# guo-research-group/Blurry-Edges

Hardware: AMD Instinct MI355X
Metric: patch-pairs/s (local CNN + render + depth) on 21x21 synth (higher is better)
Workload: dtype f32; 1 GPU; configs[1]: batch of 4096 synthetic 21x21 two-aperture patch pairs per GPU (8192 CNN patches): LocalStage inference + pass-A colour solve + depth solve; pairs_per_gpu=4096, streams=2, weights=portable-generator random init (no checkpoint offline)

## Files before the change

### blurry-edges_amd/be_hip/native.py

```python
from __future__ import annotations

import ctypes as C
import os

import torch

_HERE = os.path.dirname(os.path.abspath(__file__))
_ALT_DIR = os.environ.get("BE_LIB_DIR")
LIB_PATH = os.path.join(_ALT_DIR or os.path.join(os.path.dirname(_HERE), "lib"), "libblurry_edges_hip.so")

BE_R = 21
NPIX = 441
NTENSORS = 86


class PackJob(C.Structure):
    _fields_ = [("weight", C.c_void_p), ("bias", C.c_void_p), ("bn_gamma", C.c_void_p), ("bn_beta", C.c_void_p),
                ("bn_mean", C.c_void_p), ("bn_var", C.c_void_p), ("packed_w", C.c_void_p), ("packed_bias", C.c_void_p),
                ("bn_eps", C.c_float), ("cout", C.c_int), ("cin", C.c_int), ("ksize", C.c_int), ("layout_chw_hw", C.c_int),
                ("dgrad", C.c_int)]


class AdamEntry(C.Structure):
    _fields_ = [("p", C.c_void_p), ("m", C.c_void_p), ("v", C.c_void_p), ("goff", C.c_int64), ("n", C.c_int)]
# ... 57 lines not shown
    "be_conv_nhwc_splitk_f32": (C.c_int, [C.POINTER(ConvDesc), _P, _P, _P, _P, _P, C.c_int, _P, C.c_size_t, _P]),
    "be_conv_nhwc_batched_f32": (C.c_int, [C.POINTER(ConvDesc), _P, _P, _P, _P, C.c_int, C.c_int, C.c_int64, C.c_int64, C.c_int64, _P]),
    "be_wino_tile_rows": (C.c_int, []),
    "be_wino_packed_floats": (C.c_size_t, [C.c_int, C.c_int]),
    "be_wino_pack_f32": (C.c_int, [_P] * 6 + [C.c_float, C.c_int, C.c_int, _P, _P, _P]),
    "be_wino_workspace_floats": (C.c_size_t, [C.c_int64, C.c_int, C.c_int]),
    "be_wino_conv3x3_6x6_f32": (C.c_int, [_P] * 5 + [C.c_int64, C.c_int, C.c_int, C.c_int, _P, C.c_size_t, _P]),
    "be_gemm_rows_bf6_packed_floats": (C.c_size_t, [C.c_int, C.c_int]),
    "be_gemm_rows_bf6_pack_f32": (C.c_int, [_P, C.c_int, C.c_int, _P, _P]),
    "be_gemm_rows_bf6_f32": (C.c_int, [_P, C.c_int64, C.c_int, _P, C.c_int, _P, _P, C.c_int, _P, C.c_int, _P]),
    "be_conv3x3_pm_bf6_packed_floats": (C.c_size_t, [C.c_int, C.c_int, C.c_int]),
    "be_conv3x3_pm_bf6_pack_f32": (C.c_int, [_P, C.c_int, C.c_int, C.c_int, _P, _P]),
    "be_conv3x3_pm_bf6_f32": (C.c_int, [C.POINTER(ConvDesc), _P, _P, C.c_int, _P, _P, _P, C.c_int, _P]),
    "be_wino_pair_workspace_floats": (C.c_size_t, [C.c_int64, C.c_int, C.c_int, C.c_int]),
    "be_wino_conv3x3_pair_6x6_f32": (C.c_int, [_P, _P, _P, C.c_int, _P, _P, _P, C.c_int, _P, C.c_int64, C.c_int, C.c_int, C.c_int, _P,
                                               C.c_size_t, _P]),
    "be_conv_fused2_packed_floats": (C.c_size_t, [C.c_int] * 4),
    "be_conv_pack_fused2_f32": (C.c_int, [_P] * 12 + [C.c_float] + [C.c_int] * 4 + [_P, _P, _P]),
    "be_conv_nhwc_fused2_f32": (C.c_int, [C.POINTER(ConvDesc), _P, _P, C.c_int, _P, _P, _P, C.c_int, _P]),
    "be_maxpool_nhwc_f32": (C.c_int, [_P, _P] + [C.c_int] * 7 + [_P]),
    "be_eval_depth_f32": (C.c_int, [_P, _P, _P] + [C.c_int] * 4 + [C.c_float] * 3 + [_P, _P]),
    "be_maxpool_nhwc_ld_f32": (C.c_int, [_P, C.c_int, _P] + [C.c_int] * 7 + [_P]),
    "be_nchw_to_nhwc_pad_f32": (C.c_int, [_P, _P, C.c_int64, C.c_int, C.c_int64, C.c_int, _P]),
    "be_upconv2x2_scatter_f32": (C.c_int, [_P, _P, C.c_int64] + [C.c_int] * 9 + [_P]),
    "be_datagen_raster_words": (C.c_size_t, [C.c_int] * 4),
    "be_datagen_raster_u32": (C.c_int, [_P, _P] + [C.c_int] * 4 + [_P, _P]),
    "be_datagen_scene_f64": (C.c_int, [_P, _P, _P, _P] + [C.c_int] * 4 + [C.c_double] + [_P] * 5),
    "be_datagen_blur_scratch_bytes": (C.c_size_t, [C.c_int] * 3),
    "be_datagen_blur_composite_f64": (C.c_int, [_P] * 5 + [C.c_int] * 5 + [_P, _P, C.c_size_t, _P]),
    "be_datagen_finish_f64": (C.c_int, [_P] * 4 + [C.c_int] * 3 + [_P, C.c_size_t, _P]),
    "be_datagen_noise_f64": (C.c_int, [_P, _P, C.c_double, C.c_uint32, C.c_int64, C.c_int64, _P, _P, _P]),
    "be_datagen_candidates_f64": (C.c_int, [_P, _P] + [C.c_int] * 5 + [_P]),
    "be_datagen_crop_f64": (C.c_int, [_P, _P, _P, _P, _P, C.c_int64] + [C.c_int] * 4 + [_P, _P]),
    "be_datagen_test_psf_doubles": (C.c_size_t, [C.c_int] * 3),
    "be_datagen_test_render_f64": (C.c_int, [_P] * 8 + [C.c_size_t] + [C.c_int] * 6 + [_P, _P, _P]),
    "be_attention_train_workspace_floats": (C.c_size_t, [C.c_int, C.c_int, C.c_int]),
    "be_attention_train_fwd_f32": (C.c_int, [_P, _P, _P, _P, C.c_int, C.c_int, C.c_int, C.c_int, C.c_float, C.c_uint32, _P]),
    "be_attention_bwd_scratch_floats": (C.c_size_t, [C.c_int, C.c_int, C.c_int]),
    "be_attention_bwd_f32": (C.c_int, [_P, _P, _P, _P, _P, _P, _P, C.c_int, C.c_int, C.c_int, C.c_int, C.c_int, C.c_float, C.c_uint32, _P]),
    "be_attention_dropout_mask_f32": (C.c_int, [_P, C.c_int, C.c_int, C.c_int, C.c_float, C.c_uint32, _P]),
    "be_attention_train_keep_offset_floats": (C.c_size_t, [C.c_int, C.c_int, C.c_int]),
    "be_attention_keep_bits_u16": (C.c_int, [_P, C.c_int, C.c_int, C.c_int, C.c_float, C.c_uint32, _P]),
    "be_dropout_f32": (C.c_int, [_P, _P, _P, C.c_int64, C.c_float, C.c_uint32, C.c_uint32, _P]),
    "be_add_layernorm_train_f32": (C.c_int, [_P, _P, _P, _P, _P, _P, C.c_int64, C.c_int, C.c_float, C.c_float, C.c_uint32,
                                             C.c_uint32, _P]),
    "be_layernorm_bwd_partial_floats": (C.c_size_t, [C.c_int64, C.c_int]),
    "be_layernorm_bwd_f32": (C.c_int, [_P, _P, _P, _P, _P, _P, C.c_int64, C.c_int, C.c_float, C.c_float, C.c_uint32,
                                       C.c_uint32, _P]),
    "be_nchw3_to_nhwc4_f32": (C.c_int, [_P, _P, C.c_int64, C.c_int, _P]),
    "be_nchw3_to_nhwc4p_f32": (C.c_int, [_P, _P, C.c_int64, C.c_int, C.c_int, C.c_int, _P]),
    "be_view_to_nhwc4p_f32": (C.c_int, [_P, C.c_int64, C.c_int64, _P, C.c_int64, C.c_int, _P]),
    "be_conv7x7_nhwc4p_f32": (C.c_int, [C.POINTER(ConvDesc), _P, C.c_int, _P, _P, _P, C.c_int, _P]),
    "be_conv7x7_pool_nhwc4p_f32": (C.c_int, [_P, C.c_int64, _P, _P, _P, _P]),
    "be_render_full_f32": (C.c_int, [C.POINTER(RenderOpts), C.POINTER(DepthConsts), C.c_float, C.c_int, _P,
                                     C.POINTER(PatchView), _P, _P, _P, _P, _P, _P, _P, C.c_int64, _P]),
    "be_fold_records_f32": (C.c_int, [C.POINTER(RenderOpts), _P] + [C.c_int] * 6 + [_P] * 6 + [_P]),
    "be_fold_records_batch_f32": (C.c_int, [C.POINTER(RenderOpts), _P] + [C.c_int] * 7 + [_P] * 6 + [_P]),
    "be_render_full_grid_f32": (C.c_int, [C.POINTER(RenderOpts), C.POINTER(DepthConsts), C.c_float, C.c_int, _P, _P, C.c_int, C.c_int,
                                          _P, _P, C.c_int, C.c_int, _P, _P]),
    "be_fold_records_grid_f32": (C.c_int, [C.POINTER(RenderOpts), _P] + [C.c_int] * 4 + [_P, _P, C.c_int] + [_P] * 6 + [_P]),
    "be_refocus_stack_chunk": (C.c_int, []),
    "be_fold_refocus_stack_f32": (C.c_int, [C.POINTER(RenderOpts), C.POINTER(DepthConsts), _P] + [C.c_int] * 5 + [_P, _P, _P, C.c_int, _P, _P]),
    "be_fold_records_at_f32": (C.c_int, [C.POINTER(RenderOpts), _P] + [C.c_int] * 5 + [_P, _P] + [C.c_int] * 6 + [_P] * 6 + [_P]),
    "be_fold_refocus_stack_at_f32": (C.c_int, [C.POINTER(RenderOpts), C.POINTER(DepthConsts), _P] + [C.c_int] * 5 + [_P, _P] + [C.c_int] * 5
                                     + [_P, C.c_int, _P, _P]),
    "be_fold_records_points_f32": (C.c_int, [C.POINTER(RenderOpts), _P] + [C.c_int] * 5 + [_P, _P, _P, C.c_int64, C.c_int] + [_P] * 6 + [_P]),
    "be_fold_refocus_stack_points_f32": (C.c_int, [C.POINTER(RenderOpts), C.POINTER(DepthConsts), _P] + [C.c_int] * 5
                                         + [_P, _P, _P, C.c_int64, _P, C.c_int, _P, _P]),
    "be_unproject_f32": (C.c_int, [_P] + [C.c_int] * 5 + [C.POINTER(C.c_float)] * 2 + [_P, _P]),
    "be_reproject_f32": (C.c_int, [_P] + [C.c_int] * 5 + [C.POINTER(C.c_float)] * 3 + [C.c_float, C.c_int, C.c_int, _P, C.c_int] + [_P] * 4 + [_P]),
    "be_fill_nearest_f32": (C.c_int, [_P, _P, C.c_int, C.c_int, C.c_int, C.c_float, C.c_int] + [_P] * 4 + [_P]),
    "be_unfold_patches_f32": (C.c_int, [_P, _P] + [C.c_int] * 5 + [_P]),
    "be_local_features_f32": (C.c_int, [_P, _P, _P, C.c_int64, _P]),
    "be_global_denorm_f32": (C.c_int, [_P, _P, C.c_int64, _P]),
    "be_local_loss_f32": (C.c_int, [C.POINTER(RenderOpts), _P, _P, _P, _P, _P, C.c_float, C.c_float, _P, _P, _P, _P,
                                    C.c_int64, _P]),
    "be_train_scratch_bytes": (C.c_size_t, []),
    "be_bn_train_fwd_f32": (C.c_int, [_P, _P, _P, _P, C.c_float, C.c_float, _P, _P, _P, _P, _P, _P, C.c_int, C.c_int,
                                      C.c_int, _P, C.c_size_t, _P]),
    "be_bn_train_bwd_f32": (C.c_int, [_P] * 10 + [C.c_int, C.c_int, _P, C.c_size_t, _P]),
    "be_col_sum_f32": (C.c_int, [_P, _P, C.c_int, C.c_int, _P, C.c_size_t, _P]),
    "be_maxpool_nhwc_bwd_f32": (C.c_int, [_P, _P, _P] + [C.c_int] * 7 + [_P]),
    "be_conv_wgrad_f32": (C.c_int, [_P, _P, _P] + [C.c_int] * 7 + [_P, C.c_size_t, _P]),
    "be_conv_dgrad_packed_floats": (C.c_size_t, [C.c_int, C.c_int, C.c_int]),
    "be_conv_pack_dgrad_f32": (C.c_int, [_P, C.c_int, C.c_int, C.c_int, C.c_int, _P, _P, _P]),
    "be_linear_small_bwd_f32": (C.c_int, [_P] * 6 + [C.c_int] * 3 + [_P]),
    "be_adam_chunk": (C.c_int, []),
    "be_clip_adamw_f32": (C.c_int, [_P, C.c_int, _P, C.c_int64, _P, C.c_int, C.c_float, C.c_float] + [C.c_double] * 5 + [_P, _P, C.c_int, _P]),
    "be_local_loss_finish_f32": (C.c_int, [_P, C.c_int, C.c_float, C.c_float, _P, _P]),
    "be_train_unit_fwd_f32": (C.c_int, [_P] * 7 + [C.c_float, C.c_float] + [_P] * 7 + [C.c_int, _P, C.c_size_t, _P]),
    "be_train_unit_bwd_f32": (C.c_int, [_P] * 11 + [C.c_int] + [_P] * 8 + [C.c_size_t, _P]),
    "be_train_unit_pair_fwd_f32": (C.c_int, [C.POINTER(TrainUnitFwd), C.POINTER(TrainUnitFwd), C.c_float, C.c_float, _P, C.c_size_t, _P]),
    "be_train_unit_pair_bwd_f32": (C.c_int, [C.POINTER(TrainUnitBwd), C.POINTER(TrainUnitBwd), _P, C.c_size_t, _P]),
    "be_train_sk_plan_debug": (C.c_int, [C.c_int] * 7 + [C.c_double, C.POINTER(C.c_int), C.c_int]),
    "be_linear_param_grads_f32": (C.c_int, [_P, _P, _P, _P, C.c_int, C.c_int, C.c_int, _P, C.c_size_t, _P]),
    "be_linear_small_fwd_f32": (C.c_int, [_P] * 4 + [C.c_int] * 3 + [_P]),
    "be_maxpool_nhwc_fwd_idx_f32": (C.c_int, [_P, _P, _P] + [C.c_int] * 7 + [_P]),
    "be_maxpool_nhwc_bwd_idx_f32": (C.c_int, [_P, _P, _P] + [C.c_int] * 7 + [_P]),
    "be_params2dists_f32": (C.c_int, [C.POINTER(RenderOpts), _P, _P, C.c_int64, _P]),
    "be_dists2indicators_f32": (C.c_int, [_P, _P, _P, C.c_int64, _P]),
    "be_inverse3x3_f32": (C.c_int, [_P, _P, C.c_int64, _P]),
    "be_image_derivative_f32": (C.c_int, [_P, _P, C.c_int64, C.c_int, C.c_int, _P]),
    "be_fold_patches_f32": (C.c_int, [_P, _P, _P] + [C.c_int] * 7 + [C.c_int64] * 6 + [C.c_int, _P]),
    "be_params2dists_bwd_f32": (C.c_int, [C.POINTER(RenderOpts), _P, _P, _P, C.c_int64, _P]),
    "be_dists2indicators_bwd_f32": (C.c_int, [_P, _P, _P, _P, _P, C.c_int64, _P]),
    "be_inverse3x3_bwd_f32": (C.c_int, [_P, _P, _P, C.c_int64, _P]),
# ... 404 lines not shown
    check(lib().be_upconv2x2_scatter_f32(dptr(t, "t"), dptr(out, "out"), n, h, w, cout, oh, ow, (oh - 2 * h) // 2,
                                         (ow - 2 * w) // 2, ld, ch_off, stream_ptr(t.device)), "be_upconv2x2_scatter_f32")
    return out


def nchw3_to_nhwc4(x):
    n, c, h, w = x.shape
    if c != 3:
        raise RuntimeError("nchw3_to_nhwc4: expected 3 channels")
    y = torch.empty(n, h, w, 4, dtype=torch.float32, device=x.device)
    check(lib().be_nchw3_to_nhwc4_f32(dptr(x, "x"), dptr(y), n, h * w, stream_ptr(x.device)), "be_nchw3_to_nhwc4_f32")
    return y


def patches_to_nhwc4(x):
    n, c, h, w = x.shape
    if c == 3 and (h, w) == (BE_R, BE_R) and x.dtype == torch.float32 and n > 0 and x.stride() == (h * w * 3, 1, w * 3, 3):
        dptr(x.permute(0, 2, 3, 1), "x")
        view = PatchView(x.data_ptr(), 0, 1, w * 3, 3, 0, h * w * 3, n)
        y = torch.empty(n, h, w, 4, dtype=torch.float32, device=x.device)
        check(lib().be_view_to_nhwc4_f32(C.byref(view), n, 0, dptr(y), n, stream_ptr(x.device)), "be_view_to_nhwc4_f32")
        return y
    return nchw3_to_nhwc4(x.to(torch.float32).contiguous())


def nchw3_to_nhwc4p(x, wrow=28):
    n, c, h, w = x.shape
    if c != 3:
        raise RuntimeError("nchw3_to_nhwc4p: expected 3 channels")
    y = torch.empty(n, h, wrow, 4, dtype=torch.float32, device=x.device)
    check(lib().be_nchw3_to_nhwc4p_f32(dptr(x, "x"), dptr(y), n, h, w, wrow, stream_ptr(x.device)), "be_nchw3_to_nhwc4p_f32")
    return y


def conv7x7_nhwc4p(xp, w_img, pw, pb, cout, act):
    n, h, wrow, c4 = xp.shape
    y = torch.empty(n, h, w_img, cout, dtype=torch.float32, device=xp.device)
    d = ConvDesc(n, h, w_img, 4, cout, 7, int(act))
    check(lib().be_conv7x7_nhwc4p_f32(C.byref(d), dptr(xp, "x"), wrow, dptr(pw), dptr(pb), dptr(y), cout, stream_ptr(xp.device)),
          "be_conv7x7_nhwc4p_f32")
    return y


def conv7x7_pool_nhwc4p(xp, pw, pb):
    n, h, wrow, c4 = xp.shape
    if (h, wrow, c4) != (21, 28, 4):
        raise RuntimeError(f"conv7x7_pool_nhwc4p: expected [N,21,28,4], got {tuple(xp.shape)}")
    y = torch.empty(n, 11, 11, 64, dtype=torch.float32, device=xp.device)
    check(lib().be_conv7x7_pool_nhwc4p_f32(dptr(xp, "x"), n, dptr(pw), dptr(pb), dptr(y), stream_ptr(xp.device)),
          "be_conv7x7_pool_nhwc4p_f32")
    return y


def local_stage_pack(tensors, eps=1e-5):
    if len(tensors) != NTENSORS:
        raise RuntimeError(f"local_stage_pack: expected {NTENSORS} tensors, got {len(tensors)}")
    o = ops()
    if o is not None:
        return o.local_stage_pack(list(tensors), float(eps))
    keep = [t.contiguous() for t in tensors]
    arr = (_P * NTENSORS)(*[dptr(t, f"tensor[{i}]") for i, t in enumerate(keep)])
    dev = keep[0].device
    packed = torch.empty(lib().be_local_stage_packed_floats(), dtype=torch.float32, device=dev)
    check(lib().be_local_stage_pack_f32(arr, eps, dptr(packed), stream_ptr(dev)), "be_local_stage_pack_f32")
    return packed


class LocalStageOpts(C.Structure):
    _fields_ = [("winograd", C.c_int), ("chunk", C.c_int)]


def local_stage_forward(packed, x, out=None, workspace=None, winograd=True, chunk=0):
    n = x.shape[0]
    if tuple(x.shape[1:]) != (3, BE_R, BE_R):
        raise RuntimeError(f"LocalStage input must be [N,3,21,21], got {tuple(x.shape)}")
    dev = x.device
    o = ops()
    if o is not None:
        return o.local_stage_forward(packed, x, out, workspace, bool(winograd), int(chunk))
    if out is None:
        out = torch.empty(n, 10, dtype=torch.float32, device=dev)
    need = lib().be_local_stage_workspace_bytes(n, int(chunk))
    if workspace is None or workspace.numel() * 4 < need:
        workspace = torch.empty((need + 3) // 4, dtype=torch.float32, device=dev)
    opts = LocalStageOpts(int(bool(winograd)), int(chunk))
    check(lib().be_local_stage_forward_f32(dptr(packed, "packed"), dptr(x, "x"), dptr(out), n, dptr(workspace),
                                           workspace.numel() * 4, C.byref(opts), stream_ptr(dev)), "be_local_stage_forward_f32")
    return out, workspace


def wino_pack(weight, bias, bn=None, eps=1e-5):
    cout, cin = weight.shape[0], weight.shape[1]
    nfl = lib().be_wino_packed_floats(cout, cin)
    if nfl == 0 or tuple(weight.shape[2:]) != (3, 3):
        raise RuntimeError(f"wino_pack: unsupported conv shape {tuple(weight.shape)}")
    dev = weight.device
    pw = torch.empty(nfl, dtype=torch.float32, device=dev)
    pb = torch.empty((cout + 31) // 32 * 32, dtype=torch.float32, device=dev)
    g = bn if bn is not None else (None, None, None, None)
    check(lib().be_wino_pack_f32(dptr(weight.contiguous(), "weight"), dptr(bias), dptr(g[0]), dptr(g[1]), dptr(g[2]), dptr(g[3]), eps,
                                 cout, cin, dptr(pw), dptr(pb), stream_ptr(dev)), "be_wino_pack_f32")
    return pw, pb


def gemm_rows_bf6_pack(pw, cout, cin):
    nfl = lib().be_gemm_rows_bf6_packed_floats(cout, cin)
# ... 28 lines not shown
    d = ConvDesc(n, h, w, cin, cout, 3, int(act))
    check(lib().be_conv3x3_pm_bf6_f32(C.byref(d), dptr(x, "x"), dptr(x2), 0 if x2 is None else x2.shape[-1], dptr(planes), dptr(pb),
                                      dptr(y), y.shape[-1], stream_ptr(x.device)), "be_conv3x3_pm_bf6_f32")
    return y


def wino_conv3x3(x, pw, pb, cout, act=0, residual=None, workspace=None):
    n, h, w, cin = x.shape
    if (h, w) != (6, 6):
        raise RuntimeError(f"wino_conv3x3: 6x6 maps only, got {h}x{w}")
    need = lib().be_wino_workspace_floats(n, cin, cout)
    if workspace is None or workspace.numel() < need:
        workspace = torch.empty(need, dtype=torch.float32, device=x.device)
    y = torch.empty(n, 6, 6, cout, dtype=torch.float32, device=x.device)
    check(lib().be_wino_conv3x3_6x6_f32(dptr(x, "x"), dptr(pw), dptr(pb), dptr(residual), dptr(y), n, cin, cout, int(act),
                                        dptr(workspace), workspace.numel(), stream_ptr(x.device)), "be_wino_conv3x3_6x6_f32")
    return y, workspace


def wino_conv3x3_pair(x, pw1, pb1, cmid, pw2, pb2, cout, act1=1, act2=1, residual=None, workspace=None):
    n_, h, w, cin = x.shape
    need = lib().be_wino_pair_workspace_floats(n_, cin, cmid, cout)
    if workspace is None or workspace.numel() < need:
        workspace = torch.empty(need, dtype=torch.float32, device=x.device)
    y = torch.empty(n_, 6, 6, cout, dtype=torch.float32, device=x.device)
    check(lib().be_wino_conv3x3_pair_6x6_f32(dptr(x, "x"), dptr(pw1), dptr(pb1), int(act1), dptr(pw2), dptr(pb2), dptr(residual),
                                             int(act2), dptr(y), n_, cin, cmid, cout, dptr(workspace), workspace.numel(),
                                             stream_ptr(x.device)), "be_wino_conv3x3_pair_6x6_f32")
    return y, workspace


def local_stage_forward_view(packed, view, patches_per_image: int, n: int, device, out=None, workspace=None, winograd=True,
                             chunk=0):
    if out is None:
        out = torch.empty(n, 10, dtype=torch.float32, device=device)
    need = lib().be_local_stage_workspace_bytes(n, int(chunk))
    if workspace is None or workspace.numel() * 4 < need:
        workspace = torch.empty((need + 3) // 4, dtype=torch.float32, device=device)
    opts = LocalStageOpts(int(bool(winograd)), int(chunk))
    check(lib().be_local_stage_forward_view_f32(dptr(packed, "packed"), C.byref(view), patches_per_image, dptr(out), n,
                                                dptr(workspace), workspace.numel() * 4, C.byref(opts), stream_ptr(device)),
          "be_local_stage_forward_view_f32")
    return out, workspace


KERNEL_NAMES = {0: "k_conv_igemm<2,2,2,2,TAPS> (128x128)", 1: "k_conv_igemm<4,1,1,3,TAPS> (128x96)",
                2: "k_conv_igemm<4,1,1,2,TAPS> (128x64)", 3: "k_conv_igemm<4,1,1,1,TAPS> (128x32)",
                4: "k_conv_igemm<4,1,1,2,ROW8> (conv1)", 5: "k_conv_igemm small-M tiles (64x64 / 128x32)",
                6: "k_wino_gemm<0, 1> (128x128 tiles, the Winograd transform-domain GEMMs of a layer - one per position: 40 for the 8x5 tiles - per launch, in split-bf16 arithmetic: six v_mfma_f32_32x32x16_bf16 per product, FLOPs counted as fp32 products; BE_WINO_F32=1: the fp32 k_wino_gemm_ws / k_wino_gemm / batched k_conv_igemm)",
                7: "row GEMMs: k_wino_gemm_ps<EPI> on pre-split weights (split-bf16 arithmetic, FLOPs counted as fp32 products: LocalStage's 1x1 downsamples and fc.1; BE_ROWS_F32=1 / BE_WINO_F32=1: fp32) and the fp32 k_wino_gemm<1> / k_wino_gemm_ws<.., 1> (1x1 convolutions / linears of large batches)",
                8: "k_wino_in / k_wino_out_in / k_wino_out / k_wino_out_pool2 (Winograd transforms)", 9: "k_maxpool_nhwc",
                10: "k_render_colors (pass A)", 11: "conv1 input staging",
                12: "k_unit_gemms / k_unit_gemms_sk (training units: weight-gradient GEMMs + data-gradient convolutions of one or two units in one launch; a residual block's two forward convolutions)",
                13: "k_conv1_pool (conv1 7x7 + Smish + max-pool 3/2/1 in one image-major kernel)"}
HBM_KERNEL_IDS = (8, 9, 10, 11)


def profile_enable(max_launches: int):
    check(lib().be_profile_enable(int(max_launches)), "be_profile_enable")


def profile_reset():
    lib().be_profile_reset()


def profile_read(cap: int):
    ids = (C.c_int * cap)(); fl = (C.c_double * cap)(); by = (C.c_double * cap)(); ms = (C.c_float * cap)()
    fx = (C.c_double * cap)()
    n = lib().be_profile_read(ids, fl, by, fx, ms, cap)
    if n < 0:
        check(n, "be_profile_read")
    return [(ids[i], fl[i], by[i], ms[i], fx[i]) for i in range(n)]



def view_image_pair(img: torch.Tensor, stride: int = 2, window=None) -> PatchView:
    if img.dim() != 4 or img.shape[0] != 2 or img.shape[1] != 3:
        raise RuntimeError(f"view_image_pair: expected [2,3,H,W], got {tuple(img.shape)}")
    dptr(img, "img")
    _, _, h, w = img.shape
    top, left, bh, bw = window if window is not None else (0, 0, h, w)
    if top < 0 or left < 0 or top + bh > h or left + bw > w or bh < BE_R or bw < BE_R:
        raise RuntimeError(f"view_image_pair: window {window} outside the {h}x{w} image")
    return PatchView(img.data_ptr() + 4 * (top * w + left), 3 * h * w, h * w, w, 1, stride * w, stride,
                     (bw - BE_R) // stride + 1)


def view_flat_patches(pat: torch.Tensor, wp: int) -> PatchView:
    if pat.dim() != 5 or pat.shape[0] != 2 or tuple(pat.shape[2:]) != (3, BE_R, BE_R):
        raise RuntimeError(f"view_flat_patches: expected [2,P,3,21,21], got {tuple(pat.shape)}")
    dptr(pat, "patches")
    p = pat.shape[1]
    return PatchView(pat.data_ptr(), 3 * NPIX * p, NPIX, BE_R, 1, 3 * NPIX * wp, 3 * NPIX, wp)


def view_unfolded(t: torch.Tensor) -> PatchView:
    if t.dim() != 6 or t.shape[0] != 2 or tuple(t.shape[1:4]) != (3, BE_R, BE_R):
        raise RuntimeError(f"view_unfolded: expected [2,3,21,21,Hp,Wp], got {tuple(t.shape)}")
    dptr(t, "img_patches")
    hp, wp = t.shape[4], t.shape[5]
    p = hp * wp
    return PatchView(t.data_ptr(), 3 * NPIX * p, NPIX * p, BE_R * p, p, wp, 1, wp)


RENDER_EXTRAS = ("patches", "shpd", "refoc", "boundary", "depth_map", "depth_mask")


# ... 567 lines not shown
```

### blurry-edges_amd/csrc/be_common.h

```cpp
#pragma once
#include <hip/hip_runtime.h>
#include <atomic>
#include <cstdarg>
#include <cstdio>
#include "../../include/blurry_edges_hip.h"

namespace be {

char* last_error_buf();

inline int fail(int code, const char* fmt, ...) {
    va_list ap;
    va_start(ap, fmt);
    vsnprintf(last_error_buf(), 512, fmt, ap);
    va_end(ap);
    return code;
}

inline int check_launch(const char* what) {
    hipError_t e = hipGetLastError();
    if (e != hipSuccess) return fail(BE_ELAUNCH, "%s: %s", what, hipGetErrorString(e));
    return BE_OK;
}

inline hipStream_t as_stream(void* s) { return reinterpret_cast<hipStream_t>(s); }

constexpr int kMaxDevices = 64;
inline int current_device() {
    int d = 0;
    if (hipGetDevice(&d) != hipSuccess || d < 0 || d >= kMaxDevices) d = 0;
    return d;
}

struct DeviceFlags { std::atomic<int> v[kMaxDevices]; };
inline int ensure_dynamic_lds(const void* kernel, size_t lds_bytes, DeviceFlags& flags) {
    const int dev = current_device();
    if (flags.v[dev].load(std::memory_order_acquire)) return BE_OK;
    hipError_t e = hipFuncSetAttribute(kernel, hipFuncAttributeMaxDynamicSharedMemorySize, (int)lds_bytes);
    if (e != hipSuccess) return fail(BE_ELAUNCH, "hipFuncSetAttribute: %s", hipGetErrorString(e));
    flags.v[dev].store(1, std::memory_order_release);
    return BE_OK;
}
inline int device_cu_count() {
    static DeviceFlags cus{};
    const int dev = current_device();
    int c = cus.v[dev].load(std::memory_order_acquire);
    if (c > 0) return c;
    if (hipDeviceGetAttribute(&c, hipDeviceAttributeMultiprocessorCount, dev) != hipSuccess || c <= 0) c = 256;
    cus.v[dev].store(c, std::memory_order_release);
    return c;
}

inline bool aligned16(const void* p) { return (reinterpret_cast<uintptr_t>(p) & 15u) == 0; }

struct ProfileScope {
    ProfileScope(hipStream_t s, int kernel_id, double flops, double bytes, double flops_executed);
    ~ProfileScope();
    hipStream_t s_; int slot_;
};

int gemm_rows(const float* x, int64_t M, int K, const float* packed_w, int N, const float* bias, const float* res, int act,
              float* y, int ldy, void* stream);

int gemm_rows_ws(const float* x, int64_t M, int K, const float* packed_w, int N, float* y, int ldy, void* stream);
int gemm_rows_bf6(const float* x, int64_t M, int K, const float* planes, int N, const float* bias, const float* res, int act,
                  float* y, int ldy, void* stream);
bool rows_bf6_enabled();
int vec_add_inplace(float* a, const float* b, int n, void* stream);

int conv_pm(const be_conv_desc* d, const float* x, int wrow, const float* x2, int cin2, const float* pw, const float* pb,
            float* y, int ldy, int ktot, void* stream);

int conv3x3_pm_bf6(const be_conv_desc* d, const float* x, const float* x2, int cin2, const float* planes, const float* bias,
                   float* y, int ldy, void* stream);
bool l0_bf6_enabled();

int wino_pair(const float* x, const float* packed_w1, const float* packed_bias1, int act1, const float* packed_w2,
              const float* packed_bias2, const float* residual, int act2, float* y, int64_t n, int cin, int cmid, int cout,
              float* workspace, size_t workspace_floats, void* stream, int pool2);
int conv_train(const be_conv_desc* d, const float* x, const float* pw, const float* pb, const float* res, float* y, int ldy,
               void* scratch, size_t scratch_bytes, int* S_out, int* ldp_out, void* stream);

#define BE_REQUIRE(cond, ...) do { if (!(cond)) return be::fail(BE_EINVAL, __VA_ARGS__); } while (0)

}
```

### blurry-edges_amd/csrc/be_local_stage.hip

```cpp
#include "be_common.h"
#include <cstdlib>
#include <initializer_list>

namespace {

struct LayerSpec { int cout, cin, ks, chw_hw; };
constexpr LayerSpec kLayers[15] = {
    {64, 3, 7, 0},
    {96, 64, 3, 0},   {96, 96, 3, 0},   {96, 64, 1, 0},
    {256, 96, 3, 0},  {256, 256, 3, 0}, {256, 96, 1, 0},
    {384, 256, 3, 0}, {384, 384, 3, 0}, {384, 256, 1, 0},
    {256, 384, 3, 0}, {256, 256, 3, 0}, {256, 384, 1, 0},
    {1024, 2304, 1, 9},
    {10, 1024, 1, 0},
};

inline size_t cout_pad(int c) { return (size_t)((c + 31) / 32 * 32); }

struct PackedLayout {
    size_t w_off[15], b_off[15], total;
    size_t uw_off[15], ub_off[15];
    size_t dw_off[15], db_off[15];
    PackedLayout() {
        size_t o = 0;
// ... 129 lines not shown
    d.cin = kLayers[2].cin;
    return be::conv3x3_pm_bf6(&d, t, x, kLayers[3].cin, packed + L.sw_off[2], packed + L.b_off[2], o, 96, stream);
}

int block_wino(const float* packed, int l0, const float* x, float* t, float* o, float* r, float* w, int n, void* stream, int pool2 = 0) {
    const PackedLayout& L = layout();
    const int c = kLayers[l0].cout;
    (void)t;
    if (be::rows_bf6_enabled()) {
        if (int rc = be::gemm_rows_bf6(x, (int64_t)n * 36, kLayers[l0 + 2].cin, packed + L.sw_off[l0 + 2], c, nullptr, nullptr, 0, r, c,
                                       stream)) return rc;
    } else {
        int rc = be::gemm_rows_ws(x, (int64_t)n * 36, kLayers[l0 + 2].cin, packed + L.dw_off[l0 + 2], c, r, c, stream);
        if (rc < 0) return rc;
        if (rc > 0) {
            be_conv_desc d;
            d.n = n; d.h = 6; d.w = 6; d.cin = kLayers[l0 + 2].cin; d.cout = c; d.ksize = 1; d.act = 0;
            if ((rc = be_conv_nhwc_f32(&d, x, packed + L.dw_off[l0 + 2], packed + L.zero_off, nullptr, r, c, stream))) return rc;
        }
    }
    return be::wino_pair(x, packed + L.uw_off[l0], packed + L.ub_off[l0], 1, packed + L.uw_off[l0 + 1], packed + L.ub_off[l0 + 1], r,
                         1, o, n, kLayers[l0].cin, c, c, w, (size_t)n * RW, stream, pool2);
}

}

namespace {

int forward_impl(const float* packed, const float* x, const be_patch_view* view, int64_t P, float* out, int64_t n,
                 void* workspace, size_t workspace_bytes, const be_local_stage_opts* opts, void* stream, const char* who) {
    BE_REQUIRE(n >= 0, "%s: n < 0", who);
    BE_REQUIRE(!opts || opts->chunk >= 0, "%s: opts->chunk < 0", who);
    const int g_wino = opts ? (opts->winograd != 0) : 1;
    const int g_chunk = chunk_of(opts ? opts->chunk : 0);
    if (n == 0) return BE_OK;
    BE_REQUIRE(packed && (x || view) && out && workspace, "%s: null pointer", who);
    BE_REQUIRE(be::aligned16(workspace) && be::aligned16(packed), "%s: workspace / packed must be 16-byte aligned", who);
    if (workspace_bytes < be_local_stage_workspace_bytes(n, g_chunk))
        return be::fail(BE_EWORKSPACE, "%s: workspace %zu B < %zu B needed", who, workspace_bytes,
                        be_local_stage_workspace_bytes(n, g_chunk));
    float* ws = static_cast<float*>(workspace);
    for (int64_t first = 0; first < n; first += g_chunk) {
        const int nb = (int)((n - first) < g_chunk ? (n - first) : g_chunk);
        float* ra = ws;
        float* rb = ra + (size_t)nb * RA;
        float* rc_ = rb + (size_t)nb * RB;
        float* rw = rc_ + (size_t)nb * RC;
        float* rr = rw + (size_t)nb * RW;
        const bool wino = g_wino != 0;
        int rc;
        float* x4 = rb;
        float* p1 = rb + (size_t)nb * 1764 * 2;
        static const bool no_pm = getenv("BE_NO_CONV_PM") != nullptr;
        bool pooled = false;
        if (nb >= 512 && !no_pm) {
            if (x) rc = be_nchw3_to_nhwc4p_f32(x + first * 3 * BE_NPIX, x4, nb, BE_R, BE_R, 28, stream);
            else rc = be_view_to_nhwc4p_f32(view, P, first, x4, nb, 28, stream);
            if (rc) return rc;
            const PackedLayout& L = layout();
            static const bool no_c1p = getenv("BE_NO_CONV1_POOL") != nullptr;
            if (!no_c1p) {
                if ((rc = be_conv7x7_pool_nhwc4p_f32(x4, nb, packed + L.w_off[0], packed + L.b_off[0], p1, stream))) return rc;
                pooled = true;
            } else {
                be_conv_desc d;
                d.n = nb; d.h = 21; d.w = 21; d.cin = 4; d.cout = 64; d.ksize = 7; d.act = 1;
                if ((rc = be_conv7x7_nhwc4p_f32(&d, x4, 28, packed + L.w_off[0], packed + L.b_off[0], ra, 64, stream))) return rc;
            }
        } else {
            if (x) rc = be_nchw3_to_nhwc4_f32(x + first * 3 * BE_NPIX, x4, nb, BE_NPIX, stream);
            else rc = be_view_to_nhwc4_f32(view, P, first, x4, nb, stream);
            if (rc) return rc;
            if ((rc = conv(packed, 0, x4, nullptr, ra, nb, 21, 1, 64, stream))) return rc;
        }
        if (!pooled && (rc = be_maxpool_nhwc_f32(ra, p1, nb, 21, 21, 64, 3, 2, 1, stream))) return rc;
        if ((rc = (wino && be::l0_bf6_enabled()) ? block_l0_bf6(packed, p1, ra, rc_, nb, stream)
                                                 : block(packed, 1, p1, ra, rc_, nb, 11, stream))) return rc;
        float* p2 = rb;
        if ((rc = be_maxpool_nhwc_f32(rc_, p2, nb, 11, 11, 96, 3, 2, 1, stream))) return rc;
        if ((rc = wino ? block_wino(packed, 4, p2, ra, rc_, rr, rw, nb, stream) : block(packed, 4, p2, ra, rc_, nb, 6, stream))) return rc;
        if ((rc = wino ? block_wino(packed, 7, rc_, ra, rb, rr, rw, nb, stream) : block(packed, 7, rc_, ra, rb, nb, 6, stream))) return rc;
        float* p3;
        if (wino) {
            p3 = rc_;
            if ((rc = block_wino(packed, 10, rb, ra, p3, rr, rw, nb, stream, 1))) return rc;
        } else {
            if ((rc = block(packed, 10, rb, ra, rc_, nb, 6, stream))) return rc;
            p3 = rb;
            if ((rc = be_maxpool_nhwc_f32(rc_, p3, nb, 6, 6, 256, 2, 2, 0, stream))) return rc;
        }
        float* f1 = ra;
        if (wino && be::rows_bf6_enabled()) {
            const PackedLayout& L = layout();
            if ((rc = be::gemm_rows_bf6(p3, nb, 2304, packed + L.sw_off[13], 1024, packed + L.b_off[13], nullptr, 1, f1, 1024, stream)))
                return rc;
        } else if ((rc = conv(packed, 13, p3, nullptr, f1, nb, 1, 1, 1024, stream))) return rc;
        if ((rc = conv(packed, 14, f1, nullptr, out + first * BE_LOCAL_OUT, nb, 1, 0, BE_LOCAL_OUT, stream))) return rc;
    }
    return BE_OK;
}

}

extern "C" int be_local_stage_forward_f32(const float* packed, const float* x, float* out, int64_t n,
                                          void* workspace, size_t workspace_bytes, const be_local_stage_opts* opts, void* stream) {
    BE_REQUIRE(x || n == 0, "be_local_stage_forward_f32: null pointer");
    return forward_impl(packed, x, nullptr, 1, out, n, workspace, workspace_bytes, opts, stream, "be_local_stage_forward_f32");
}

extern "C" int be_local_stage_forward_view_f32(const float* packed, const be_patch_view* view, int64_t patches_per_image,
                                               float* out, int64_t n, void* workspace, size_t workspace_bytes,
                                               const be_local_stage_opts* opts, void* stream) {
    BE_REQUIRE((view && view->base && view->wp > 0 && patches_per_image > 0) || n == 0,
               "be_local_stage_forward_view_f32: bad view");
// ... 4 lines not shown
```

### blurry-edges_amd/csrc/be_split_bf16.h

```cpp
#pragma once
#include <hip/hip_runtime.h>

namespace be {
namespace bf6 {

typedef float f32x4 __attribute__((ext_vector_type(4)));
typedef float f32x2 __attribute__((ext_vector_type(2)));
typedef __bf16 bf16x8 __attribute__((ext_vector_type(8)));
typedef __bf16 bf16x2 __attribute__((ext_vector_type(2)));

__device__ __forceinline__ float bf_lo(unsigned u) { return __uint_as_float(u << 16); }
__device__ __forceinline__ float bf_hi(unsigned u) { return __uint_as_float(u & 0xffff0000u); }
__device__ __forceinline__ float sub_f32(float x, float y) {
    float r;
    asm("v_sub_f32 %0, %1, %2" : "=v"(r) : "v"(x), "v"(y));
    return r;
}
__device__ __forceinline__ void split8(f32x4 a, f32x4 b, bf16x8& h, bf16x8& m, bf16x8& l) {
    const float x[8] = {a.x, a.y, a.z, a.w, b.x, b.y, b.z, b.w};
#pragma unroll
    for (int e = 0; e < 8; e += 2) {
        const bf16x2 hb = __builtin_convertvector((f32x2){x[e], x[e + 1]}, bf16x2);
        const unsigned hu = __builtin_bit_cast(unsigned, hb);
        const float r0 = sub_f32(x[e], bf_lo(hu)), r1 = sub_f32(x[e + 1], bf_hi(hu));
        const bf16x2 mb = __builtin_convertvector((f32x2){r0, r1}, bf16x2);
        const unsigned mu = __builtin_bit_cast(unsigned, mb);
        const bf16x2 lb = __builtin_convertvector((f32x2){sub_f32(r0, bf_lo(mu)), sub_f32(r1, bf_hi(mu))}, bf16x2);
        h[e] = hb[0]; h[e + 1] = hb[1];
        m[e] = mb[0]; m[e + 1] = mb[1];
        l[e] = lb[0]; l[e + 1] = lb[1];
    }
}

constexpr int PS_BLOCK = 3 * 128 * 16;
__device__ __forceinline__ int ps_slot(int row, int half) { return half ^ ((row >> 3) & 1); }

}
}
```

### include/blurry_edges_hip.h

```cpp
#ifndef BLURRY_EDGES_HIP_H
#define BLURRY_EDGES_HIP_H

#include <stddef.h>
#include <stdint.h>

#ifdef __cplusplus
extern "C" {
#endif

#define BE_OK            0
#define BE_EINVAL       -1
#define BE_EWORKSPACE   -2
#define BE_ELAUNCH      -3

#define BE_R             21
#define BE_NPIX          441
#define BE_LOCAL_OUT     10

int         be_version(void);
const char* be_last_error(void);


typedef struct be_depth_consts {
    float s;
// ... 169 lines not shown
    float bn_eps;
    int cout, cin, ksize, layout_chw_hw, dgrad;
} be_pack_job;
int be_conv_pack_jobs_f32(const be_pack_job* jobs_device, int njobs, void* stream);
int be_conv_nhwc_f32(const be_conv_desc* desc_host, const float* x, const float* packed_w,
                     const float* packed_bias, const float* residual, float* y, int ldy, void* stream);
int be_conv_nhwc_splitk_f32(const be_conv_desc* d, const float* x, const float* packed_w, const float* packed_bias,
                            const float* residual, float* y, int ldy, void* scratch, size_t scratch_bytes, void* stream);
size_t be_conv_fused2_packed_floats(int cout, int cin, int ksize, int cin2);
int be_conv_pack_fused2_f32(const float* weight_oihw, const float* bias, const float* bn_gamma, const float* bn_beta,
                            const float* bn_mean, const float* bn_var, const float* weight2_oi, const float* bias2,
                            const float* bn2_gamma, const float* bn2_beta, const float* bn2_mean, const float* bn2_var,
                            float bn_eps, int cout, int cin, int ksize, int cin2, float* packed_w, float* packed_bias,
                            void* stream);
int be_conv_nhwc_fused2_f32(const be_conv_desc* desc_host, const float* x, const float* x2, int cin2,
                            const float* packed_w, const float* packed_bias, float* y, int ldy, void* stream);
int be_conv_nhwc_batched_f32(const be_conv_desc* d, const float* x, const float* packed_w, const float* packed_bias, float* y,
                             int ldy, int nbatch, int64_t x_stride, int64_t w_stride, int64_t y_stride, void* stream);

int be_wino_tile_rows(void);
size_t be_wino_packed_floats(int cout, int cin);
int be_wino_pack_f32(const float* w_oihw, const float* bias, const float* bn_gamma, const float* bn_beta, const float* bn_mean,
                     const float* bn_var, float bn_eps, int cout, int cin, float* packed_w, float* packed_bias, void* stream);
size_t be_wino_workspace_floats(int64_t n, int cin, int cout);
int be_wino_conv3x3_6x6_f32(const float* x, const float* packed_w, const float* packed_bias, const float* residual, float* y,
                            int64_t n, int cin, int cout, int act, float* workspace, size_t workspace_floats, void* stream);

size_t be_wino_pair_workspace_floats(int64_t n, int cin, int cmid, int cout);
int be_wino_conv3x3_pair_6x6_f32(const float* x, const float* packed_w1, const float* packed_bias1, int act1,
                                 const float* packed_w2, const float* packed_bias2, const float* residual, int act2, float* y,
                                 int64_t n, int cin, int cmid, int cout, float* workspace, size_t workspace_floats, void* stream);

size_t be_gemm_rows_bf6_packed_floats(int cout, int cin);
int be_gemm_rows_bf6_pack_f32(const float* packed_w, int cout, int cin, float* planes, void* stream);
int be_gemm_rows_bf6_f32(const float* x, int64_t m, int k, const float* planes, int n, const float* bias, const float* residual,
                         int act, float* y, int ldy, void* stream);

size_t be_conv3x3_pm_bf6_packed_floats(int cout, int cin, int cin2);
int be_conv3x3_pm_bf6_pack_f32(const float* packed_w, int cout, int cin, int cin2, float* planes, void* stream);
int be_conv3x3_pm_bf6_f32(const be_conv_desc* desc_host, const float* x, const float* x2, int cin2, const float* planes,
                          const float* packed_bias, float* y, int ldy, void* stream);

int be_maxpool_nhwc_f32(const float* x, float* y, int n, int h, int w, int c, int k, int stride, int pad,
                        void* stream);
int be_maxpool_nhwc_ld_f32(const float* x, int ldx, float* y, int n, int h, int w, int c, int k, int stride, int pad,
                           void* stream);
int be_nchw3_to_nhwc4_f32(const float* x, float* y, int64_t n, int hw, void* stream);
int be_nchw3_to_nhwc4p_f32(const float* x, float* y, int64_t n, int h, int w, int wrow, void* stream);
int be_view_to_nhwc4p_f32(const be_patch_view* view_host, int64_t patches_per_image, int64_t first, float* y, int64_t n,
                          int wrow, void* stream);
int be_conv7x7_nhwc4p_f32(const be_conv_desc* d, const float* x, int wrow, const float* packed_w, const float* packed_bias,
                          float* y, int ldy, void* stream);
int be_conv7x7_pool_nhwc4p_f32(const float* x4p, int64_t n, const float* packed_w, const float* packed_bias, float* y, void* stream);
int be_view_to_nhwc4_f32(const be_patch_view* view_host, int64_t patches_per_image, int64_t first, float* y,
                         int64_t n, void* stream);

size_t be_train_scratch_bytes(void);
int be_bn_train_fwd_f32(const float* y, const float* gamma, const float* beta, const float* res, float eps,
                        float momentum, float* run_mean, float* run_var, float* mean, float* invstd, float* s_in,
                        float* out, int M, int C, int act, void* scratch, size_t scratch_bytes, void* stream);
int be_bn_train_bwd_f32(const float* dout, const float* s_in, const float* y, const float* mean, const float* invstd,
                        const float* gamma, float* ds, float* dy, float* dgamma, float* dbeta, int M, int C,
                        void* scratch, size_t scratch_bytes, void* stream);
int be_col_sum_f32(const float* a, float* out, int M, int C, void* scratch, size_t scratch_bytes, void* stream);
int be_maxpool_nhwc_bwd_f32(const float* x, const float* dout, float* dx, int n, int h, int w, int c, int k, int stride,
                            int pad, void* stream);
int be_conv_wgrad_f32(const float* x, const float* dy, float* dw, int n, int h, int w, int cin, int cout, int ksize,
                      int layout_chw_hw, void* scratch, size_t scratch_bytes, void* stream);
size_t be_conv_dgrad_packed_floats(int cout, int cin, int ksize);
int be_conv_pack_dgrad_f32(const float* weight_oihw, int cout, int cin, int ksize, int layout_chw_hw, float* packed_w,
                           float* packed_bias, void* stream);
int be_linear_small_bwd_f32(const float* x, const float* w, const float* dy, float* dx, float* dw, float* db, int M,
                            int K, int J, void* stream);

int be_train_unit_fwd_f32(const be_conv_desc* desc_host, const float* x, const float* packed_w, const float* packed_bias,
                          const float* gamma, const float* beta, const float* res, float eps, float momentum, float* run_mean,
                          float* run_var, float* y, float* mean, float* invstd, float* s_in, float* out, int act,
                          void* scratch, size_t scratch_bytes, void* stream);
int be_train_unit_bwd_f32(const be_conv_desc* desc_host, const float* x, const float* dout, const float* s_in, const float* y,
                          const float* mean, const float* invstd, const float* gamma, const float* dgrad_packed_w,
                          const float* dgrad_packed_bias, const float* dx_add, int layout_chw_hw, float* ds, float* dy,
                          float* dgamma, float* dbeta, float* dw, float* db, float* dx, void* scratch, size_t scratch_bytes,
                          void* stream);
typedef struct be_train_unit_fwd {
    be_conv_desc desc;
    const float *x, *packed_w, *packed_bias, *gamma, *beta, *res;
    float *run_mean, *run_var, *y, *mean, *invstd, *s_in, *out;
    int act;
} be_train_unit_fwd;
typedef struct be_train_unit_bwd {
    be_conv_desc desc;
    const float *x, *dout, *s_in, *y, *mean, *invstd, *gamma, *dgrad_packed_w, *dgrad_packed_bias, *dx_add;
    int layout_chw_hw;
    float *ds, *dy, *dgamma, *dbeta, *dw, *db, *dx;
} be_train_unit_bwd;
int be_train_unit_pair_fwd_f32(const be_train_unit_fwd* a, const be_train_unit_fwd* b, float eps, float momentum,
                               void* scratch, size_t scratch_bytes, void* stream);
int be_train_unit_pair_bwd_f32(const be_train_unit_bwd* a, const be_train_unit_bwd* b, void* scratch, size_t scratch_bytes,
                               void* stream);
int be_train_sk_plan_debug(int n, int h, int w, int cin, int cout, int ksize, int workgroups, double w_share, int* seg, int cap);

int be_linear_param_grads_f32(const float* x, const float* dy, float* dw, float* db, int M, int cin, int cout, void* scratch,
                              size_t scratch_bytes, void* stream);
int be_linear_small_fwd_f32(const float* x, const float* w, const float* b, float* y, int M, int K, int J, void* stream);
int be_maxpool_nhwc_fwd_idx_f32(const float* x, float* y, unsigned char* idx, int n, int h, int w, int c, int k, int stride,
                                int pad, void* stream);
// ... 91 lines not shown
```

Measured before the change: 431,800 patch-pairs/s.

## Add split-bf16 MFMA conv1 7x7 + Smish + max-pool kernel with LDS pre-split image

Adds a new fused conv1+Smish+maxpool kernel that runs the 7x7 convolution on MFMA 32x32x16 bf16 instructions using three-way split-bf16 (six MFMAs per product) to approximate fp32 accuracy. The input image is split into hi/mid/lo bf16 planes once in LDS, the next image is prefetched into registers while the current one computes, and pooling uses LDS atomic fmax. It becomes the default path whenever the Winograd path is enabled, also for batches below 512, replacing the fp32 FMA conv1_pool kernel. This trades scalar fp32 FMA throughput for matrix-core throughput at the cost of six times as many products and slightly different rounding.

Result: faster. 456,300 patch-pairs/s (median of 6 runs) (+5.7%).

```diff
diff --git a/blurry-edges_amd/be_hip/native.py b/blurry-edges_amd/be_hip/native.py
--- a/blurry-edges_amd/be_hip/native.py
+++ b/blurry-edges_amd/be_hip/native.py
@@ -133,6 +133,7 @@
     "be_view_to_nhwc4p_f32": (C.c_int, [_P, C.c_int64, C.c_int64, _P, C.c_int64, C.c_int, _P]),
     "be_conv7x7_nhwc4p_f32": (C.c_int, [C.POINTER(ConvDesc), _P, C.c_int, _P, _P, _P, C.c_int, _P]),
     "be_conv7x7_pool_nhwc4p_f32": (C.c_int, [_P, C.c_int64, _P, _P, _P, _P]),
+    "be_conv7x7_pool_bf6_nhwc4p_f32": (C.c_int, [_P, C.c_int64, _P, _P, _P, _P]),
     "be_render_full_f32": (C.c_int, [C.POINTER(RenderOpts), C.POINTER(DepthConsts), C.c_float, C.c_int, _P,
                                      C.POINTER(PatchView), _P, _P, _P, _P, _P, _P, _P, C.c_int64, _P]),
     "be_fold_records_f32": (C.c_int, [C.POINTER(RenderOpts), _P] + [C.c_int] * 6 + [_P] * 6 + [_P]),
@@ -643,6 +644,16 @@
     return y
 
 
+def conv7x7_pool_bf6_nhwc4p(xp, pw, pb):
+    n, h, wrow, c4 = xp.shape
+    if (h, wrow, c4) != (21, 28, 4):
+        raise RuntimeError(f"conv7x7_pool_bf6_nhwc4p: expected [N,21,28,4], got {tuple(xp.shape)}")
+    y = torch.empty(n, 11, 11, 64, dtype=torch.float32, device=xp.device)
+    check(lib().be_conv7x7_pool_bf6_nhwc4p_f32(dptr(xp, "x"), n, dptr(pw), dptr(pb), dptr(y), stream_ptr(xp.device)),
+          "be_conv7x7_pool_bf6_nhwc4p_f32")
+    return y
+
+
 def local_stage_pack(tensors, eps=1e-5):
     if len(tensors) != NTENSORS:
         raise RuntimeError(f"local_stage_pack: expected {NTENSORS} tensors, got {len(tensors)}")
@@ -777,7 +788,7 @@
                 8: "k_wino_in / k_wino_out_in / k_wino_out / k_wino_out_pool2 (Winograd transforms)", 9: "k_maxpool_nhwc",
                 10: "k_render_colors (pass A)", 11: "conv1 input staging",
                 12: "k_unit_gemms / k_unit_gemms_sk (training units: weight-gradient GEMMs + data-gradient convolutions of one or two units in one launch; a residual block's two forward convolutions)",
-                13: "k_conv1_pool (conv1 7x7 + Smish + max-pool 3/2/1 in one image-major kernel)"}
+                13: "k_conv1_pool_bf6 (conv1 7x7 + Smish + max-pool 3/2/1 in one image-major kernel, in split-bf16 arithmetic with the image pre-split in LDS, FLOPs counted as fp32 products; BE_C1_F32=1 / BE_WINO_F32=1: the fp32 k_conv1_pool)"}
 HBM_KERNEL_IDS = (8, 9, 10, 11)
 
 
diff --git a/blurry-edges_amd/csrc/be_common.h b/blurry-edges_amd/csrc/be_common.h
--- a/blurry-edges_amd/csrc/be_common.h
+++ b/blurry-edges_amd/csrc/be_common.h
@@ -74,6 +74,7 @@
 int conv3x3_pm_bf6(const be_conv_desc* d, const float* x, const float* x2, int cin2, const float* planes, const float* bias,
                    float* y, int ldy, void* stream);
 bool l0_bf6_enabled();
+bool c1_bf6_enabled();
 
 int wino_pair(const float* x, const float* packed_w1, const float* packed_bias1, int act1, const float* packed_w2,
               const float* packed_bias2, const float* residual, int act2, float* y, int64_t n, int cin, int cmid, int cout,
diff --git a/blurry-edges_amd/csrc/be_conv1_pool_bf6.hip b/blurry-edges_amd/csrc/be_conv1_pool_bf6.hip
--- /dev/null
+++ b/blurry-edges_amd/csrc/be_conv1_pool_bf6.hip
@@ -0,0 +1,194 @@
+#include "be_common.h"
+#include "be_device_math.h"
+#include "be_split_bf16.h"
+#include <cstdlib>
+
+namespace {
+
+using be::bf6::bf16x4;
+using be::bf6::bf16x8;
+using be::bf6::f32x4;
+using be::bf6::split4;
+using be::bf6::split8;
+typedef float f32x16 __attribute__((ext_vector_type(16)));
+typedef unsigned u32x2 __attribute__((ext_vector_type(2)));
+typedef unsigned u32x4 __attribute__((ext_vector_type(4)));
+typedef const volatile __attribute__((address_space(3))) u32x2* lds_frag_t;
+
+constexpr int R = 21, HW = R * R, WROW = 28, PADR = R + 6, COUT = 64, KTOT = 224, OR_ = 11;
+constexpr int LROW = 53;
+constexpr int PLANE_BYTES = PADR * LROW * 8;
+constexpr int IMG_BYTES = (3 * PLANE_BYTES + 15) / 16 * 16;
+constexpr int IMG_QUADS = R * WROW;
+constexpr int POOL_FLOATS = OR_ * OR_ * COUT;
+constexpr int CELL = COUT + 16;
+constexpr int POOL_LDS = OR_ * OR_ * CELL;
+constexpr size_t LDS_BYTES = (size_t)IMG_BYTES + POOL_LDS * sizeof(float);
+static_assert(2 * LDS_BYTES <= 160 * 1024, "two workgroups per CU");
+static_assert(3 * PLANE_BYTES + 6 * LROW * 8 + 64 < 65536, "fragment offsets are 16-bit immediates");
+
+__device__ __forceinline__ void lds_fmax(float* p, float v) {
+    __builtin_amdgcn_ds_fmaxf((__attribute__((address_space(3))) float*)p, v, __ATOMIC_RELAXED, __MEMORY_SCOPE_WRKGRP, false);
+}
+
+__global__ __launch_bounds__(256, 2)
+void k_conv1_pool_bf6(const float* __restrict__ x4p, const float* __restrict__ w, const float* __restrict__ bias, float* __restrict__ y,
+                      int64_t n) {
+    extern __shared__ __attribute__((aligned(16))) float smem_c1b[];
+    char* const img_lds = reinterpret_cast<char*>(smem_c1b);
+    const __attribute__((address_space(3))) char* const img3 = (const __attribute__((address_space(3))) char*)img_lds;
+    float* pool = smem_c1b + IMG_BYTES / 4;
+    const int tid = threadIdx.x;
+    const int wave = tid >> 6, lane = tid & 63, li = lane & 31, lh = lane >> 5;
+    const int ntile = wave & 1, mpar = wave >> 1;
+    const int cout = ntile * 32 + li;
+
+    for (int i = tid; i < IMG_BYTES / 16; i += 256) reinterpret_cast<f32x4*>(img_lds)[i] = f32x4{0.f, 0.f, 0.f, 0.f};
+    bf16x8 bw[14][3];
+#pragma unroll
+    for (int c = 0; c < 14; ++c) {
+        const float* wp = w + (size_t)cout * KTOT + (c >> 1) * 32 + (c & 1) * 16 + lh * 8;
+        split8(*reinterpret_cast<const f32x4*>(wp), *reinterpret_cast<const f32x4*>(wp + 4), bw[c][0], bw[c][1], bw[c][2]);
+    }
+    const float bs = bias ? bias[cout] : 0.0f;
+    for (int i = tid; i < POOL_LDS / 4; i += 256) reinterpret_cast<f32x4*>(pool)[i] = f32x4{-INFINITY, -INFINITY, -INFINITY, -INFINITY};
+
+    int64_t img = blockIdx.x;
+    f32x4 pre[3];
+    auto fetch = [&](int64_t im) {
+        const f32x4* src = reinterpret_cast<const f32x4*>(x4p + im * (int64_t)(R * WROW * 4));
+#pragma unroll
+        for (int j = 0; j < 3; ++j) {
+            const int q = tid + 256 * j;
+            pre[j] = q < IMG_QUADS ? src[q] : f32x4{0.f, 0.f, 0.f, 0.f};
+        }
+    };
+    auto stash = [&]() {
+#pragma unroll
+        for (int j = 0; j < 3; ++j) {
+            const int q = tid + 256 * j;
+            if (q < IMG_QUADS) {
+                bf16x4 h, m, l;
+                split4(pre[j], h, m, l);
+                char* dst = img_lds + ((q / WROW + 3) * LROW + q % WROW) * 8;
+                *reinterpret_cast<bf16x4*>(dst) = h;
+                *reinterpret_cast<bf16x4*>(dst + PLANE_BYTES) = m;
+                *reinterpret_cast<bf16x4*>(dst + 2 * PLANE_BYTES) = l;
+            }
+        }
+    };
+    __syncthreads();
+    if (img < n) { fetch(img); stash(); }
+    __syncthreads();
+
+    for (; img < n; img += gridDim.x) {
+        const int64_t nxt = img + gridDim.x;
+        if (nxt < n) fetch(nxt);
+#pragma unroll 1
+        for (int s = 0; s < 7; ++s) {
+            const int t0 = mpar + 2 * s;
+            const int p0 = min(t0 * 32 + li, HW - 1);
+            const int py0 = (p0 * 3121) >> 16, px0_ = p0 - py0 * R;
+            unsigned o0 = (unsigned)((py0 * LROW + px0_ + 2 * lh) * 8);
+            unsigned o1 = o0 + 8;
+            unsigned o2 = lh ? (unsigned)((py0 * LROW + WROW) * 8) : o0 + 40;
+            asm("" : "+v"(o1));
+            asm("" : "+v"(o2));
+            auto frag = [&](int c, bf16x8 (&f)[3]) {
+                const int kh = c >> 1, half = c & 1;
+#pragma unroll
+                for (int p = 0; p < 3; ++p) {
+                    const int off = p * PLANE_BYTES + kh * LROW * 8;
+                    const u32x2 a = *reinterpret_cast<lds_frag_t>(img3 + o0 + off + half * 32);
+                    const u32x2 b = *reinterpret_cast<lds_frag_t>(img3 + (half ? o2 : o1) + off);
+                    f[p] = __builtin_bit_cast(bf16x8, (u32x4){a.x, a.y, b.x, b.y});
+                }
+            };
+            f32x16 acc;
+#pragma unroll
+            for (int r = 0; r < 16; ++r) acc[r] = 0.f;
+            bf16x8 fa[3];
+            frag(0, fa);
+#pragma unroll
+            for (int c = 0; c < 14; ++c) {
+                bf16x8 fn[3];
+                if (c + 1 < 14) frag(c + 1, fn);
+                constexpr int PA[6] = {2, 0, 1, 1, 0, 0}, PB[6] = {0, 2, 1, 0, 1, 0};
+#pragma unroll
+                for (int p = 0; p < 6; ++p) acc = __builtin_amdgcn_mfma_f32_32x32x16_bf16(fa[PA[p]], bw[c][PB[p]], acc, 0, 0, 0);
+                if (c + 1 < 14) {
+#pragma unroll
+                    for (int p = 0; p < 3; ++p) fa[p] = fn[p];
+                }
+            }
+#pragma unroll
+            for (int c4 = 0; c4 < 4; ++c4) {
+                const int qb = t0 * 32 + 8 * c4 + 4 * lh;
+                if (qb >= HW) continue;
+                float v[4];
+#pragma unroll
+                for (int e = 0; e < 4; ++e) v[e] = be::smish(acc[4 * c4 + e] + bs);
+                const int py = (qb * 3121) >> 16, px0 = qb - py * R;
+                if (px0 + 3 < R) {
+                    const int a_ = px0 >> 1;
+                    float ma, mb, mc;
+                    if (px0 & 1) { ma = v[0]; mb = fmaxf(v[0], fmaxf(v[1], v[2])); mc = fmaxf(v[2], v[3]); }
+                    else { ma = fmaxf(v[0], v[1]); mb = fmaxf(v[1], fmaxf(v[2], v[3])); mc = v[3]; }
+                    float* c = pool + ((py >> 1) * OR_ + a_) * CELL + cout;
+                    lds_fmax(c, ma); lds_fmax(c + CELL, mb); lds_fmax(c + 2 * CELL, mc);
+                    if (py & 1) { c += OR_ * CELL; lds_fmax(c, ma); lds_fmax(c + CELL, mb); lds_fmax(c + 2 * CELL, mc); }
+                } else {
+#pragma unroll
+                    for (int e = 0; e < 4; ++e) {
+                        const int q = qb + e;
+                        if (q >= HW) continue;
+                        const int qy = (q * 3121) >> 16, qx = q - qy * R;
+                        float* c = pool + ((qy >> 1) * OR_ + (qx >> 1)) * CELL + cout;
+                        lds_fmax(c, v[e]);
+                        if (qx & 1) lds_fmax(c + CELL, v[e]);
+                        if (qy & 1) {
+                            lds_fmax(c + OR_ * CELL, v[e]);
+                            if (qx & 1) lds_fmax(c + (OR_ + 1) * CELL, v[e]);
+                        }
+                    }
+                }
+            }
+        }
+        __syncthreads();
+        float* yo = y + img * (int64_t)POOL_FLOATS;
+        for (int i = tid; i < POOL_FLOATS / 4; i += 256) {
+            f32x4* cell = reinterpret_cast<f32x4*>(pool + (i >> 4) * CELL) + (i & 15);
+            reinterpret_cast<f32x4*>(yo)[i] = *cell;
+            *cell = f32x4{-INFINITY, -INFINITY, -INFINITY, -INFINITY};
+        }
+        if (nxt < n) stash();
+        __syncthreads();
+    }
+}
+
+}
+
+bool be::c1_bf6_enabled() {
+    static const bool f32 = (getenv("BE_C1_F32") != nullptr && atoi(getenv("BE_C1_F32")) != 0) ||
+                            (getenv("BE_WINO_F32") != nullptr && atoi(getenv("BE_WINO_F32")) != 0);
+    return !f32;
+}
+
+extern "C" int be_conv7x7_pool_bf6_nhwc4p_f32(const float* x4p, int64_t n, const float* packed_w, const float* packed_bias, float* y,
+                                              void* stream) {
+    BE_REQUIRE(x4p && packed_w && y, "be_conv7x7_pool_bf6_nhwc4p_f32: null pointer");
+    BE_REQUIRE(n > 0 && n < ((int64_t)1 << 31), "be_conv7x7_pool_bf6_nhwc4p_f32: n outside (0, 2^31)");
+    BE_REQUIRE(be::aligned16(x4p) && be::aligned16(packed_w) && be::aligned16(y), "be_conv7x7_pool_bf6_nhwc4p_f32: 16-byte alignment");
+    static be::DeviceFlags attr_set{};
+    if (int rc_ = be::ensure_dynamic_lds(reinterpret_cast<const void*>(&k_conv1_pool_bf6), LDS_BYTES, attr_set)) return rc_;
+    hipStream_t s = be::as_stream(stream);
+    const int cus = be::device_cu_count();
+    const unsigned grid = (unsigned)(n < 2 * cus ? n : 2 * cus);
+    {
+        const double M = (double)n * HW;
+        be::ProfileScope prof(s, BE_KERNEL_CONV1_POOL, 2.0 * M * 147.0 * COUT, 4.0 * (M * 3.0 + 147.0 * COUT + (double)n * OR_ * OR_ * COUT),
+                              (double)n * 14.0 * 2.0 * 14.0 * 32768.0);
+        hipLaunchKernelGGL(k_conv1_pool_bf6, dim3(grid), dim3(256), LDS_BYTES, s, x4p, packed_w, packed_bias, y, n);
+    }
+    return be::check_launch("be_conv7x7_pool_bf6_nhwc4p_f32");
+}
diff --git a/blurry-edges_amd/csrc/be_local_stage.hip b/blurry-edges_amd/csrc/be_local_stage.hip
--- a/blurry-edges_amd/csrc/be_local_stage.hip
+++ b/blurry-edges_amd/csrc/be_local_stage.hip
@@ -205,14 +205,18 @@
         float* x4 = rb;
         float* p1 = rb + (size_t)nb * 1764 * 2;
         static const bool no_pm = getenv("BE_NO_CONV_PM") != nullptr;
+        static const bool no_c1p = getenv("BE_NO_CONV1_POOL") != nullptr;
+        const bool c1_bf6 = wino && be::c1_bf6_enabled() && !no_pm && !no_c1p;
         bool pooled = false;
-        if (nb >= 512 && !no_pm) {
+        if (c1_bf6 || (nb >= 512 && !no_pm)) {
             if (x) rc = be_nchw3_to_nhwc4p_f32(x + first * 3 * BE_NPIX, x4, nb, BE_R, BE_R, 28, stream);
             else rc = be_view_to_nhwc4p_f32(view, P, first, x4, nb, 28, stream);
             if (rc) return rc;
             const PackedLayout& L = layout();
-            static const bool no_c1p = getenv("BE_NO_CONV1_POOL") != nullptr;
-            if (!no_c1p) {
+            if (c1_bf6) {
+                if ((rc = be_conv7x7_pool_bf6_nhwc4p_f32(x4, nb, packed + L.w_off[0], packed + L.b_off[0], p1, stream))) return rc;
+                pooled = true;
+            } else if (!no_c1p) {
                 if ((rc = be_conv7x7_pool_nhwc4p_f32(x4, nb, packed + L.w_off[0], packed + L.b_off[0], p1, stream))) return rc;
                 pooled = true;
             } else {
diff --git a/blurry-edges_amd/csrc/be_split_bf16.h b/blurry-edges_amd/csrc/be_split_bf16.h
--- a/blurry-edges_amd/csrc/be_split_bf16.h
+++ b/blurry-edges_amd/csrc/be_split_bf16.h
@@ -32,6 +32,23 @@
     }
 }
 
+typedef __bf16 bf16x4 __attribute__((ext_vector_type(4)));
+__device__ __forceinline__ void split4(f32x4 a, bf16x4& h, bf16x4& m, bf16x4& l) {
+    const float x[4] = {a.x, a.y, a.z, a.w};
+#pragma unroll
+    for (int e = 0; e < 4; e += 2) {
+        const bf16x2 hb = __builtin_convertvector((f32x2){x[e], x[e + 1]}, bf16x2);
+        const unsigned hu = __builtin_bit_cast(unsigned, hb);
+        const float r0 = sub_f32(x[e], bf_lo(hu)), r1 = sub_f32(x[e + 1], bf_hi(hu));
+        const bf16x2 mb = __builtin_convertvector((f32x2){r0, r1}, bf16x2);
+        const unsigned mu = __builtin_bit_cast(unsigned, mb);
+        const bf16x2 lb = __builtin_convertvector((f32x2){sub_f32(r0, bf_lo(mu)), sub_f32(r1, bf_hi(mu))}, bf16x2);
+        h[e] = hb[0]; h[e + 1] = hb[1];
+        m[e] = mb[0]; m[e + 1] = mb[1];
+        l[e] = lb[0]; l[e + 1] = lb[1];
+    }
+}
+
 constexpr int PS_BLOCK = 3 * 128 * 16;
 __device__ __forceinline__ int ps_slot(int row, int half) { return half ^ ((row >> 3) & 1); }
 
diff --git a/include/blurry_edges_hip.h b/include/blurry_edges_hip.h
--- a/include/blurry_edges_hip.h
+++ b/include/blurry_edges_hip.h
@@ -245,6 +245,7 @@
 int be_conv7x7_nhwc4p_f32(const be_conv_desc* d, const float* x, int wrow, const float* packed_w, const float* packed_bias,
                           float* y, int ldy, void* stream);
 int be_conv7x7_pool_nhwc4p_f32(const float* x4p, int64_t n, const float* packed_w, const float* packed_bias, float* y, void* stream);
+int be_conv7x7_pool_bf6_nhwc4p_f32(const float* x4p, int64_t n, const float* packed_w, const float* packed_bias, float* y, void* stream);
 int be_view_to_nhwc4_f32(const be_patch_view* view_host, int64_t patches_per_image, int64_t first, float* y,
                          int64_t n, void* stream);
 
```
